# Symb0x76/ChineseChessZero

Measured on AMD Instinct MI355X. Metric: self-play MCTS simulations/sec, higher is better.
Workload: dtype u8 rules / f32 Q (reference CPU path) / f64 PUCT (net: fp16)

## Files before the change

chinesechesszero_amd/_lib.py:

```python
from __future__ import annotations

import ctypes as C
import os

import torch

_HERE = os.path.dirname(os.path.abspath(__file__))
LIB_PATH = os.path.join(_HERE, "libcczero.so")

NSQ = 90
SQ_STRIDE = 96
NMOVES = 2086
MAX_LEGAL = 128
MASK_WORDS = 66
PLANES = 10710
REC_BYTES, REC_HDR, REC_IDS, REC_PI = 880, 96, 112, 368
HEAD_POL_STRIDE, HEAD_VAL_STRIDE = 1536, 640

ABI_VERSION = 8
CONV_RELU, CONV_DESCENDING, CONV_FORCE_SMALL, CONV_FORCE_TILE, CONV_G16, CONV_G16_EDGE_TILES = 1, 2, 16, 32, 64, 128
CONV_G16_ONE_LAUNCH = 512
RULE_PERPETUAL_CHECK = 1
RULE_PAWN_MOVE_RESETS_CLOCK = 2
FLAG_REFERENCE_QUIRKS = 1
# ... 73 lines not shown
    "ccz_gather_priors_routed": (C.c_int, [_P, _P, _P, _P, C.c_int32, _P, _P]),
    "ccz_finish_move": (C.c_int, [_P, _P, _P, _P, _P, C.c_int32]),
    "ccz_root_children": (C.c_int, [_P, _P, _P, _P, _P, _P, _P, _P]),
    "ccz_principal_variations": (C.c_int, [_P, _P, C.c_int32, C.c_int32, _P, _P, _P, _P, _P, _P]),
    "ccz_root_pi": (C.c_int, [_P, _P, _P, _P]),
    "ccz_move_distribution": (C.c_int, [_P, _P, _P, _P, _P, _P]),
    "ccz_game_status": (C.c_int, [_P, _P, _P, _P, _P, _P]),
    "ccz_root_positions": (C.c_int, [_P, _P, _P]),
    "ccz_leaf_info": (C.c_int, [_P, _P, _P, _P, _P, _P]),
    "ccz_leaf_priors": (C.c_int, [_P, _P, _P, _P]),
    "ccz_leaf_keys": (C.c_int, [_P, _P, _P, _P]),
    "ccz_harvest_rows": (C.c_int, [_P, _P, C.POINTER(C.c_int64)]),
    "ccz_harvest": (C.c_int, [_P, _P, _P, _P, _P, C.c_int64, C.POINTER(C.c_int64)]),
    "ccz_harvest_records": (C.c_int, [_P, _P, _P, C.c_int64, C.POINTER(C.c_int64)]),
    "ccz_expand_records": (C.c_int, [_P, _P, C.c_int64, C.c_uint32, _P, _P, _P, _P, C.c_int64, C.c_int64, _P]),
    "ccz_ring_retire": (C.c_int, [_P, _P, C.c_int64, _P, C.c_int64, C.c_int32, _P]),
    "ccz_sample_records": (C.c_int, [_P, _P, C.c_int64, _P, _P, C.c_int64, C.c_uint32, _P, _P, _P, _P, _P]),
    "ccz_get_stats": (C.c_int, [_P, _P, C.POINTER(Stats)]),
    "ccz_legal_moves": (C.c_int, [_P, C.c_int32, _P, _P, _P, _P, _P, _P]),
    "ccz_apply_moves": (C.c_int, [_P, C.c_int32, _P, _P, _P, _P]),
    "ccz_bias_act_f16": (C.c_int, [_P, _P, _P, _P, C.c_int64, C.c_int32]),
    "ccz_conv3x3_c256_f16": (C.c_int, [_P, _P, _P, _P, _P, _P, C.c_int64, C.c_int32]),
    "ccz_conv3x3_stem_f16": (C.c_int, [_P, _P, _P, _P, _P, C.c_int64, C.c_int32]),
    "ccz_pack_live_planes_f16": (C.c_int, [_P, _P, _P, C.c_int32]),
    "ccz_pack_live_planes_rows_f16": (C.c_int, [_P, _P, _P, C.c_int32, _P, _P]),
    "ccz_pack_live_planes_g16_f16": (C.c_int, [_P, _P, _P, C.c_int32, _P, _P]),
    "ccz_pack_conv_weights_g16_f16": (C.c_int, [_P, _P, _P, C.c_int32]),
    "ccz_conv3x3_c256_f16_live": (C.c_int, [_P, _P, _P, _P, _P, _P, C.c_int64, C.c_int32, _P, C.c_int32, C.c_int32]),
    "ccz_conv3x3_stem_f16_live": (C.c_int, [_P, _P, _P, _P, _P, C.c_int64, C.c_int32, _P, C.c_int32, C.c_int32]),
    "ccz_conv3x3_c256_heads_f16": (C.c_int, [_P, _P, _P, _P, _P, _P, _P, _P, _P, C.c_int64, C.c_int32, _P, C.c_int32, C.c_int32]),
    "ccz_heads_conv1x1_f16": (C.c_int, [_P, _P, _P, _P, _P, _P, C.c_int32, C.c_int32, _P]),
    "ccz_fc_f16": (C.c_int, [_P, _P, C.c_int32, _P, _P, _P, C.c_int32, C.c_int32, C.c_int32, C.c_int32, C.c_int32, _P]),
    "ccz_value_out_f32": (C.c_int, [_P, _P, _P, C.c_float, _P, C.c_int32, _P]),
}

_lib = None


def source_hash() -> str | None:
    import glob
    import hashlib
    csrc = os.path.join(_HERE, "csrc")
    files = sorted(glob.glob(os.path.join(csrc, "*.h")) + glob.glob(os.path.join(csrc, "*.hip")), key=os.path.basename)
    files.append(os.path.join(os.path.dirname(_HERE), "include", "cczero.h"))
    if len(files) < 2 or not all(os.path.exists(f) for f in files):
        return None
    h = hashlib.sha256()
    for f in files:
        with open(f, "rb") as fh:
            h.update(fh.read())
    return h.hexdigest()[:16]


def stale_build() -> str | None:
    if LIB_PATH != os.path.join(_HERE, "libcczero.so"):
        return None
    want = source_hash()
    if want is None:
        return None
    stamp = LIB_PATH + ".srchash"
    if not os.path.exists(stamp):
        return f"{LIB_PATH} carries no source stamp ({stamp} is missing): it was not built by the current Makefile"
    with open(stamp) as f:
        got = f.read().strip()
    if got != want:
        return f"{LIB_PATH} was built from other sources (stamp {got}, the tree hashes to {want}): a kernel was edited after the last build"
# ... 28 lines not shown
```

chinesechesszero_amd/csrc/cczero.hip:

```cpp
#include "../../include/cczero.h"

#include <hip/hip_runtime.h>

#include <cmath>
#include <cstdarg>
#include <cstdio>
#include <cstring>
#include <new>
#include <vector>

#include "cczero_kernels.h"
#include "cczero_netops.h"
#include "cczero_conv.h"
#include "cczero_conv_small.h"
#include "cczero_conv_g16.h"
#include "cczero_conv_g16e.h"
#include "cczero_heads.h"

using namespace ccz;

namespace {

thread_local char g_err[512] = "";

// ... 1052 lines not shown
}

int ccz_conv3x3_c256_heads_f16(void *stream, const void *x_dev, const void *w_dev, const void *bias_f32_dev, const void *residual_dev,
                               const void *head_w32_dev, const void *head_b32_dev, void *pol_dev, void *val_dev, int64_t n_pixels, int32_t flags,
                               const int32_t *live_rows_dev, int32_t part, int32_t n_parts)
{
    const char *who = "ccz_conv3x3_c256_heads_f16";
    if (!x_dev || !w_dev || !bias_f32_dev || !residual_dev || !head_w32_dev || !head_b32_dev || !pol_dev || !val_dev || n_pixels < 0 || n_pixels % 1440 ||
        n_pixels > (int64_t)INT32_MAX / kCvC)
        return fail(-1, "%s: bad arguments (n_pixels must be a multiple of 16 boards * 90, at most 93200 boards per call)", who);
    if (!(flags & CCZ_CONV_G16)) return fail(-1, "%s: rows must be in the group-of-16 layout (CCZ_CONV_G16)", who);
    if ((((uintptr_t)x_dev) | ((uintptr_t)w_dev) | ((uintptr_t)bias_f32_dev) | ((uintptr_t)residual_dev) | ((uintptr_t)head_w32_dev) | ((uintptr_t)head_b32_dev)) & 15)
        return fail(-1, "%s: pointers must be 16-byte aligned", who);
    if ((((uintptr_t)pol_dev) | ((uintptr_t)val_dev)) & 1) return fail(-1, "%s: outputs must be 2-byte aligned", who);
    if (live_rows_dev && (n_parts < 1 || n_parts > 256 || part < 0 || part >= n_parts)) return fail(-1, "%s: bad part / n_parts", who);
    if (n_pixels == 0) return 0;
    const int groups = (int)(n_pixels / 1440);
    const int fl = flags & 3, row0 = live_rows_dev ? (part | (n_parts << 16)) : 0;
    G5Heads ha;
    ha.w32 = (const _Float16 *)head_w32_dev;
    ha.b32 = (const float *)head_b32_dev;
    ha.pol = (_Float16 *)pol_dev;
    ha.val = (_Float16 *)val_dev;
    ha.nb = (int)(n_pixels / 90);
    hipStream_t s = (hipStream_t)stream;
#define CCZ_G16H(KERNEL_, GRID_, FLAGS_)                                                                                                \
    hipLaunchKernelGGL(KERNEL_, dim3((unsigned)(GRID_)), dim3(512), 0, s, (const _Float16 *)x_dev, (const _Float16 *)w_dev, (const float *)bias_f32_dev, \
                       (const _Float16 *)residual_dev, (_Float16 *)nullptr, (int)n_pixels, (int)(FLAGS_), 256, (const int *)live_rows_dev, row0, ha)
    if (!(flags & CCZ_CONV_G16_EDGE_TILES) || groups < 2) {
        CCZ_G16H(k_conv3x3_g16_heads, groups * 5, fl);
        HIP_TRY(hipGetLastError());
        return 0;
    }
    CCZ_G16H(k_conv3x3_g16_heads, groups * 4, fl | 4);
    HIP_TRY(hipGetLastError());
    CCZ_G16H(k_conv3x3_g16_edge_heads, 2 * ((groups + 1) / 2), fl);
    HIP_TRY(hipGetLastError());
#undef CCZ_G16H
    return 0;
}

int ccz_conv3x3_stem_f16(void *stream, const void *x64_dev, const void *w_dev, const void *bias_f32_dev, void *y_dev, int64_t n_pixels, int32_t relu)
{
    return conv3x3_launch("ccz_conv3x3_stem_f16", stream, x64_dev, w_dev, bias_f32_dev, nullptr, y_dev, n_pixels, relu, 64);
}

int ccz_conv3x3_c256_f16_live(void *stream, const void *x_dev, const void *w_dev, const void *bias_f32_dev, const void *residual_dev, void *y_dev,
                              int64_t n_pixels, int32_t relu, const int32_t *live_rows_dev, int32_t part, int32_t n_parts)
{
    if (!live_rows_dev || n_parts < 1 || n_parts > 256 || part < 0 || part >= n_parts) return fail(-1, "ccz_conv3x3_c256_f16_live: null live-row count or bad part / n_parts");
    return conv3x3_launch("ccz_conv3x3_c256_f16_live", stream, x_dev, w_dev, bias_f32_dev, residual_dev, y_dev, n_pixels, relu, 256, live_rows_dev, part | (n_parts << 16));
}

int ccz_conv3x3_stem_f16_live(void *stream, const void *x64_dev, const void *w_dev, const void *bias_f32_dev, void *y_dev, int64_t n_pixels, int32_t relu,
                              const int32_t *live_rows_dev, int32_t part, int32_t n_parts)
{
    if (!live_rows_dev || n_parts < 1 || n_parts > 256 || part < 0 || part >= n_parts) return fail(-1, "ccz_conv3x3_stem_f16_live: null live-row count or bad part / n_parts");
    return conv3x3_launch("ccz_conv3x3_stem_f16_live", stream, x64_dev, w_dev, bias_f32_dev, nullptr, y_dev, n_pixels, relu, 64, live_rows_dev, part | (n_parts << 16));
}

int ccz_pack_live_planes_rows_f16(void *stream, const void *leaf_dev, void *x64_dev, int32_t n_boards, const int32_t *rows_dev, const int32_t *n_rows_dev)
{
    if (!leaf_dev || !x64_dev || n_boards < 0 || !rows_dev || !n_rows_dev) return fail(-1, "ccz_pack_live_planes_rows_f16: bad arguments");
    if ((uintptr_t)x64_dev & 15) return fail(-1, "ccz_pack_live_planes_rows_f16: output must be 16-byte aligned");
    if (n_boards == 0) return 0;
    hipLaunchKernelGGL(k_pack_live_planes, dim3((unsigned)n_boards), dim3(kPackThreads), 0, (hipStream_t)stream, (const _Float16 *)leaf_dev, (half8_t *)x64_dev, (int)n_boards,
// ... 84 lines not shown
        const dim3 wgrid((unsigned)(8 * ((wtiles + 7) / 8)));
        if (relu & 1)
            hipLaunchKernelGGL(k_fc_wide_f16<true>, wgrid, dim3(512), 0, (hipStream_t)stream, (const _Float16 *)a_dev, (int)lda, (const _Float16 *)w_dev,
                               (const float *)bias_f32_dev, (_Float16 *)c_dev, (int)ldc, (int)m, (int)n, (int)k, (const int *)live_rows_dev, (int)(relu >> 8));
        else
            hipLaunchKernelGGL(k_fc_wide_f16<false>, wgrid, dim3(512), 0, (hipStream_t)stream, (const _Float16 *)a_dev, (int)lda, (const _Float16 *)w_dev,
                               (const float *)bias_f32_dev, (_Float16 *)c_dev, (int)ldc, (int)m, (int)n, (int)k, (const int *)live_rows_dev, (int)(relu >> 8));
        HIP_TRY(hipGetLastError());
        return 0;
    }
    if (m <= 16 && !(relu & 6)) {
        const dim3 sgrid((unsigned)((n + 15) / 16));
        if (relu & 1)
            hipLaunchKernelGGL(k_fc_skinny_f16<true>, sgrid, dim3(64), 0, (hipStream_t)stream, (const _Float16 *)a_dev, (int)lda, (const _Float16 *)w_dev,
                               (const float *)bias_f32_dev, (_Float16 *)c_dev, (int)ldc, (int)m, (int)n, (int)k, (const int *)live_rows_dev);
        else
            hipLaunchKernelGGL(k_fc_skinny_f16<false>, sgrid, dim3(64), 0, (hipStream_t)stream, (const _Float16 *)a_dev, (int)lda, (const _Float16 *)w_dev,
                               (const float *)bias_f32_dev, (_Float16 *)c_dev, (int)ldc, (int)m, (int)n, (int)k, (const int *)live_rows_dev);
        HIP_TRY(hipGetLastError());
        return 0;
    }
    const int tiles = ((n + kFcBN - 1) / kFcBN) * ((m + kFcBM - 1) / kFcBM);
    const dim3 grid((unsigned)(8 * ((tiles + 7) / 8)));
    if (relu & 1)
        hipLaunchKernelGGL(k_fc_f16<true>, grid, dim3(256), 0, (hipStream_t)stream, (const _Float16 *)a_dev, (int)lda, (const _Float16 *)w_dev,
                           (const float *)bias_f32_dev, (_Float16 *)c_dev, (int)ldc, (int)m, (int)n, (int)k, (const int *)live_rows_dev, (int)(relu >> 8));
    else
        hipLaunchKernelGGL(k_fc_f16<false>, grid, dim3(256), 0, (hipStream_t)stream, (const _Float16 *)a_dev, (int)lda, (const _Float16 *)w_dev,
                           (const float *)bias_f32_dev, (_Float16 *)c_dev, (int)ldc, (int)m, (int)n, (int)k, (const int *)live_rows_dev, (int)(relu >> 8));
    HIP_TRY(hipGetLastError());
    return 0;
}

int ccz_value_out_f32(void *stream, const void *h_dev, const void *w2_dev, float b2, float *v_dev, int32_t m, const int32_t *live_rows_dev)
{
    if (!h_dev || !w2_dev || !v_dev || m < 0) return fail(-1, "ccz_value_out_f32: bad arguments");
    if ((((uintptr_t)h_dev) | ((uintptr_t)w2_dev)) & 7) return fail(-1, "ccz_value_out_f32: h and w2 must be 8-byte aligned");
    if (m == 0) return 0;
    hipLaunchKernelGGL(k_value_out, dim3((unsigned)((m + 3) / 4)), dim3(256), 0, (hipStream_t)stream, (const _Float16 *)h_dev, (const _Float16 *)w2_dev, b2, v_dev,
                       (int)m, (const int *)live_rows_dev);
    HIP_TRY(hipGetLastError());
    return 0;
}

}
```

chinesechesszero_amd/csrc/cczero_conv_g16e.h:

```cpp
#pragma once
#include "cczero_conv_g16.h"

namespace ccz {

__host__ __device__ constexpr int g5e_nslab(int h) { return h == 0 ? 2 : h == 1 ? 2 : h == 2 ? 1 : 0; }
__host__ __device__ constexpr int g5e_dma(int h) { return 2 + g5e_nslab(h); }
__host__ __device__ constexpr int g5e_vmcnt(int h) { return g5e_dma(h) + g5e_dma((h + 5) % 6); }
static_assert(g5e_vmcnt(0) == 6 && g5e_vmcnt(1) == 8 && g5e_vmcnt(2) == 7 && g5e_vmcnt(3) == 5 && g5e_vmcnt(4) == 4 && g5e_vmcnt(5) == 4, "g5e_vmcnt table");
static_assert(g5e_dma(0) == 4 && g5e_dma(1) == 4 && g5e_dma(2) == 3 && g5e_dma(3) == 2 && g5e_dma(4) == 2 && g5e_dma(5) == 2,
              "17 DMA loads per chunk and thread: 5 slab pieces + 6 x 2 weight pieces");

template <int J>
__device__ __forceinline__ void g5e_step(const G5Ctx &c, cv_f32x4 (&acc)[4][9], int chunk, int &ring_rd, int &ring_wr,
                                          cv_half8 (&a0)[4], cv_half8 (&a1)[4], cv_half8 (&b)[9], int toff)
{
    constexpr int H = J % 6, BUF = J / 6;
    constexpr int Hn = (H + 1) % 6, BUFn = (H == 5) ? 1 - BUF : BUF;
    cv_half8 (&acur)[4] = (J & 1) ? a1 : a0;
    cv_half8 (&anxt)[4] = (J & 1) ? a0 : a1;
    unsigned char *const lds = c.lds;
#define G5E_CELL(N)                                                                                                       \
    {                                                                                                                     \
        if constexpr (H % 3 == 2)                                                                                         \
            b[N] = *(const cv_half8 *)(lds + c.vb[BUFn] + ((Hn / 3) * 9 + N) * 1024);                                     \
// ... 206 lines not shown
__global__ __launch_bounds__(512) void k_conv3x3_g16_edge(const _Float16 *__restrict__ X, const _Float16 *__restrict__ W,
                                                            const float *__restrict__ bias, const _Float16 *R, _Float16 *Y, int M,
                                                            int relu, int cin, const int *live_rows, int row0)
{
    __shared__ __attribute__((aligned(16))) unsigned char lds[kG5Lds];
    g5e_tile<RES, false>(lds, blockIdx.x, X, W, bias, R, Y, M, relu, cin, live_rows, row0, G5Heads{});
}

__global__ __launch_bounds__(512) void k_conv3x3_g16_edge_heads(const _Float16 *__restrict__ X, const _Float16 *__restrict__ W,
                                                                  const float *__restrict__ bias, const _Float16 *R, _Float16 *Y,
                                                                  int M, int relu, int cin, const int *live_rows, int row0, G5Heads ha)
{
    __shared__ __attribute__((aligned(16))) unsigned char lds[kG5Lds];
    if (live_rows) ha.nb = *live_rows;
    g5e_tile<true, true>(lds, blockIdx.x, X, W, bias, R, Y, M, relu, cin, live_rows, row0, ha);
}

template <bool RES>
__global__ __launch_bounds__(512) void k_conv3x3_g16_one(const _Float16 *__restrict__ X, const _Float16 *__restrict__ W,
                                                           const float *__restrict__ bias, const _Float16 *R, _Float16 *Y, int M,
                                                           int relu, int cin, const int *live_rows, int row0)
{
    __shared__ __attribute__((aligned(16))) unsigned char lds[kG5Lds];
    int groups = M / 1440;
    if (live_rows) {
        int first;
        groups = g5_live_groups(live_rows, row0, groups, first);
    }
    const int mid = groups * 4, blk = blockIdx.x;
    if (blk < mid) g5_tile<RES, false>(lds, blk, mid, X, W, bias, R, Y, M, relu | 4, cin, live_rows, row0, G5Heads{});
    else g5e_tile<RES, false>(lds, blk - mid, X, W, bias, R, Y, M, relu, cin, live_rows, row0, G5Heads{});
}

}
```

chinesechesszero_amd/csrc/cczero_heads.h:

```cpp
#pragma once
#include <hip/hip_runtime.h>
#include <stdint.h>

#include "cczero_conv.h"
#include "cczero_device.h"

namespace ccz {

constexpr int kHdPol = 17, kHdVal = 7;
constexpr int kHdPolStride = 1536;
constexpr int kHdValStride = 640;

template <bool G16>
__global__ __launch_bounds__(256) void k_head_conv1x1(const _Float16 *__restrict__ X, const _Float16 *__restrict__ Wh,
                                                        const float *__restrict__ bh, _Float16 *__restrict__ pol,
                                                        _Float16 *__restrict__ val, int n_boards, const int *__restrict__ live)
{
    const int lane = threadIdx.x & 63, r = lane & 15, q4 = lane >> 4;
    const int wave = blockIdx.x * 4 + (threadIdx.x >> 6), n_waves = gridDim.x * 4;
    int nb = n_boards;
    if (live) { const int l = *live; nb = l < nb ? l : nb; }
    const long n_rows = G16 ? (long)((nb + 15) >> 4) * 1440 : (long)nb * 90;
    const int n_cells = (int)((n_rows + 15) >> 4);
    if (wave >= n_cells) return;
// ... 331 lines not shown
        }
        mfmas(fa1, fb1, s_ + 3, 0, s_ + 3 < ns ? 7 : 0);
    }
    FW_STAMP(2)
    if (FC_DBG(8)) { if (acc[0][0][0] == 12345.678f) C[0] = (_Float16)1; return; }
    __builtin_amdgcn_sched_barrier(0);
    __builtin_amdgcn_s_barrier();
    __builtin_amdgcn_sched_barrier(0);
    unsigned char *tb = lds + wv * (64 * kFwERow);
#pragma unroll
    for (int j = 0; j < 4; ++j)
#pragma unroll
        for (int i = 0; i < NF; ++i) {
            float v0 = acc[i][j][0], v1 = acc[i][j][1], v2 = acc[i][j][2], v3 = acc[i][j][3];
            if (RELU) { v0 = fmaxf(v0, 0.0f); v1 = fmaxf(v1, 0.0f); v2 = fmaxf(v2, 0.0f); v3 = fmaxf(v3, 0.0f); }
            cv_half4 o;
            o[0] = (_Float16)v0; o[1] = (_Float16)v1; o[2] = (_Float16)v2; o[3] = (_Float16)v3;
            *(cv_half4 *)(tb + (j * 16 + r) * kFwERow + (i * 16 + 4 * q4) * 2) = o;
        }
    wave_sync();
    constexpr int NW = NF * 8;
#pragma unroll 4
    for (int it = 0; it < NW; ++it) {
        const int L = it * 64 + lane, row = L / NW, dw = L - row * NW;
        const int m = m0 + wm * 64 + row, n = n0 + I0 * 16 + 2 * dw;
        const uint32_t v = *(const uint32_t *)(tb + row * kFwERow + dw * 4);
        if (m < Ml && n + 1 < N) *(uint32_t *)(C + (long)m * ldc + n) = v;
    }
    FW_STAMP(3)
#undef FW_STAMP
}

template <bool RELU>
__global__ __launch_bounds__(512) void k_fc_wide_f16(const _Float16 *__restrict__ A, int lda, const _Float16 *__restrict__ W,
                                                       const float *__restrict__ bias, _Float16 *__restrict__ C, int ldc, int M, int N,
                                                       int K, const int *__restrict__ live, [[maybe_unused]] int dbg)
{
    __shared__ __attribute__((aligned(16))) unsigned char lds[kFwStages * kFwStage];
    const int tid = threadIdx.x, lane = tid & 63;
    const int wv = __builtin_amdgcn_readfirstlane(tid >> 6), wm = wv & 3, wn = wv >> 2;
    int Ml = M;
    if (live) { const int l = *live; Ml = l < Ml ? l : Ml; }
    const int mt = (Ml + kFwBM - 1) / kFwBM, nt = (N + kFwBN - 1) / kFwBN, tiles = mt * nt;
    int n0, m0;
    {
        const int b = blockIdx.x, x = b & 7, per = tiles >> 3, rem = tiles & 7;
        if ((b >> 3) >= per + (x < rem ? 1 : 0)) return;
        const int t = x * per + (x < rem ? x : rem) + (b >> 3);
        const int full = (mt >> 1) * 2 * nt;
        const int blk = t < full ? t / (2 * nt) : (mt >> 1);
        const int r_ = t < full ? t % (2 * nt) : t - full;
        const int cnt = t < full ? 2 : 1;
        n0 = (r_ / cnt) * kFwBN;
        m0 = (2 * blk + r_ % cnt) * kFwBM;
    }
    const int wrows = ((N + 127) >> 7) << 7;
    const int c = (lane & 7) ^ ((4 * (wv & 1) + (lane >> 4)) & 7), lr = lane >> 3;
    const _Float16 *src[7];
#pragma unroll
    for (int t = 0; t < 4; ++t) {
        int m = m0 + (wv + 8 * t) * 8 + lr;
        m = m < Ml ? m : Ml - 1;
        src[t] = A + (long)m * lda + c * 8;
    }
#pragma unroll
    for (int t = 0; t < 3; ++t) {
        int n = n0 + (wv + 8 * t) * 8 + lr;
        n = n < wrows ? n : wrows - 1;
        src[4 + t] = W + (long)n * K + c * 8;
    }
    if (wn == 0) fw_wave<RELU, 5, 0>(lds, src, wv, wm, lane, bias, wrows - 4, C, ldc, Ml, N, K, m0, n0, dbg);
    else fw_wave<RELU, 4, 5>(lds, src, wv, wm, lane, bias, wrows - 4, C, ldc, Ml, N, K, m0, n0, dbg);
}

__global__ __launch_bounds__(256) void k_value_out(const _Float16 *__restrict__ h, const _Float16 *__restrict__ w2, float b2,
                                                    float *__restrict__ v, int M, const int *__restrict__ live)
{
    const int lane = threadIdx.x & 63, m = blockIdx.x * 4 + (threadIdx.x >> 6);
    if (m >= M) return;
    const cv_half4 x = *(const cv_half4 *)(h + (long)m * 256 + lane * 4), w = *(const cv_half4 *)(w2 + lane * 4);
    int Ml = M;
    if (live) { const int l = *live; Ml = l < Ml ? l : Ml; }
    if (m >= Ml) return;
    float s = (float)x[0] * (float)w[0];
    s += (float)x[1] * (float)w[1];
    s += (float)x[2] * (float)w[2];
    s += (float)x[3] * (float)w[3];
    s = wave_sum_f32(s) + b2;
    if (lane == 0) v[m] = tanhf((float)(_Float16)s);
}

}
```

chinesechesszero_amd/net.py:

```python
from __future__ import annotations

import os

import numpy as np
import torch
import torch.nn.functional as F
from torch import nn

PIECES = 7
PLAYS = 17


class ResBlock(nn.Module):

    def __init__(self, num_channels=256):
        super().__init__()
        self.conv1 = nn.Conv2d(num_channels, num_channels, kernel_size=(3, 3), stride=(1, 1), padding=1)
        self.conv1_bn = nn.BatchNorm2d(num_channels)
        self.conv1_act = nn.ReLU()
        self.conv2 = nn.Conv2d(num_channels, num_channels, kernel_size=(3, 3), stride=(1, 1), padding=1)
        self.conv2_bn = nn.BatchNorm2d(num_channels)
        self.conv2_act = nn.ReLU()

    def forward(self, x):
# ... 483 lines not shown
                            f"(k_conv3x3_g16 / k_conv3x3_small serve 256-channel towers): MIOpen convolutions + one-pass epilogue")
                for i in range(0, len(self.ws), 2):
                    y = self._epilogue(F.conv2d(x, self.ws[i], None, padding=1), self.bs[i])
                    x = self._epilogue(F.conv2d(y, self.ws[i + 1], None, padding=1), self.bs[i + 1], x)
        return self._heads(x, B, g16, plan, return_logits)

    def _fused_heads_ok(self, x) -> bool:
        return bool(self.opt.fused_heads and hasattr(self, "head_w32") and x.is_cuda and x.dtype == torch.float16 and x.shape[1] == 256
                    and x.is_contiguous(memory_format=torch.channels_last))

    def _head_buffers(self, Bx, dev):
        from . import _lib
        bufs = self.__dict__.setdefault("_head_bufs", {})
        key = (Bx, dev)
        if key not in bufs:
            bufs[key] = (torch.zeros((Bx, _lib.HEAD_POL_STRIDE), dtype=torch.float16, device=dev),
                         torch.zeros((Bx, _lib.HEAD_VAL_STRIDE), dtype=torch.float16, device=dev),
                         torch.empty((Bx, 256), dtype=torch.float16, device=dev))
        return bufs[key]

    def _heads_fused(self, x, B, g16, plan, conv_done=False):
        import ctypes as C
        from . import _lib
        L = _lib.lib()
        Bx, dev = x.shape[0], x.device
        pol, val, h1 = self._head_buffers(Bx, dev)
        logits = torch.empty((B, 2086), dtype=torch.float16, device=dev)
        v = torch.empty((B,), dtype=torch.float32, device=dev)
        s = C.c_void_p(torch.cuda.current_stream(dev).cuda_stream)
        live = C.c_void_p(plan[1].data_ptr()) if plan is not None else None
        P = lambda t: C.c_void_p(t.data_ptr())
        if not conv_done:
            _lib.check(L.ccz_heads_conv1x1_f16(s, P(x), P(self.head_w32), P(self.head_b32), P(pol), P(val), Bx, _lib.CONV_G16 if g16 else 0, live))
        _lib.check(L.ccz_fc_f16(s, P(pol), _lib.HEAD_POL_STRIDE, P(self.policy_fc_wp), P(self.policy_fc_b32), P(logits), 2086, B, 2086, 1536, 0, live))
        _lib.check(L.ccz_fc_f16(s, P(val), _lib.HEAD_VAL_STRIDE, P(self.value_fc1_wp), P(self.value_fc1_b32), P(h1), 256, B, 256, 640, 1, live))
        _lib.check(L.ccz_value_out_f32(s, P(h1), P(self.value_fc2_w), self._value_b2(), P(v), B, live))
        return logits, v

    def _value_b2(self) -> float:
        b2 = self.__dict__.get("_b2")
        if b2 is None:
            b2 = self.__dict__["_b2"] = float(self.value_fc2_b.detach().float().cpu().item())
        return b2

    def _heads(self, x, B, g16, plan, return_logits, conv_done=False):
        if self._fused_heads_ok(x):
            logits, v = self._heads_fused(x, B, g16, plan, conv_done)
            if return_logits:
                return logits, v
            return torch.exp(F.log_softmax(logits.float(), dim=1)).contiguous(), v
        Bx = x.shape[0]
        rows = x.permute(0, 2, 3, 1).reshape(Bx * 90, x.shape[1])
        h = F.relu_(torch.addmm(self.head_b, rows, self.head_wT))
        if g16:
            h = h.view(Bx // 16, 90, 16, PLAYS + PIECES).permute(0, 2, 1, 3).reshape(Bx, 90, PLAYS + PIECES)[:B]
        else:
            h = h.view(B, 90, PLAYS + PIECES)
        pol = h[:, :, :PLAYS].reshape(B, 90 * PLAYS)
        val = h[:, :, PLAYS:].reshape(B, 90 * PIECES)
        logits = F.linear(pol, self.policy_fc_w, self.policy_fc_b)
        v = F.relu_(F.linear(val, self.value_fc1_w, self.value_fc1_b))
        v = torch.tanh(F.linear(v, self.value_fc2_w, self.value_fc2_b).float()).view(B)
        if return_logits:
            return logits.contiguous(), v.contiguous()
        prob = torch.exp(F.log_softmax(logits.float(), dim=1))
        return prob.contiguous(), v.contiguous()
# ... 133 lines not shown
```

include/cczero.h:

```cpp
#ifndef CCZERO_H
#define CCZERO_H

#include <stdint.h>

#ifdef __cplusplus
extern "C" {
#endif

#define CCZ_ABI_VERSION 8
#define CCZ_NSQ 90
#define CCZ_SQ_STRIDE 96
#define CCZ_NMOVES 2086
#define CCZ_MAX_LEGAL 128
#define CCZ_MASK_WORDS 66
#define CCZ_PLANES 10710


#define CCZ_RULE_PAWN_MOVE_RESETS_CLOCK 2u
#define CCZ_RULE_PERPETUAL_CHECK 1u

#define CCZ_FLAG_REFERENCE_QUIRKS 1u
#define CCZ_FLAG_NO_MIRROR 2u
#define CCZ_FLAG_VALUE_F16 4u

// ... 164 lines not shown
#define CCZ_CONV_DESCENDING 2
#define CCZ_CONV_FORCE_SMALL 16
#define CCZ_CONV_FORCE_TILE 32
#define CCZ_CONV_G16 64
#define CCZ_CONV_G16_EDGE_TILES 128
#define CCZ_CONV_G16_ONE_LAUNCH 512
int ccz_conv3x3_c256_f16(void *stream, const void *x_dev, const void *w_dev, const void *bias_f32_dev,
                         const void *residual_dev, void *y_dev, int64_t n_pixels, int32_t relu);
int ccz_pack_conv_weights_g16_f16(void *stream, const void *w_dev, void *wp_dev, int32_t cin);

int ccz_conv3x3_stem_f16(void *stream, const void *x64_dev, const void *w_dev, const void *bias_f32_dev,
                         void *y_dev, int64_t n_pixels, int32_t relu);
int ccz_pack_live_planes_f16(void *stream, const void *leaf_dev, void *x64_dev, int32_t n_boards);
int ccz_pack_live_planes_g16_f16(void *stream, const void *leaf_dev, void *x64_dev, int32_t n_boards,
                                 const int32_t *rows_dev, const int32_t *n_rows_dev);

int ccz_pack_live_planes_rows_f16(void *stream, const void *leaf_dev, void *x64_dev, int32_t n_boards,
                                  const int32_t *rows_dev, const int32_t *n_rows_dev);
int ccz_conv3x3_c256_f16_live(void *stream, const void *x_dev, const void *w_dev, const void *bias_f32_dev,
                              const void *residual_dev, void *y_dev, int64_t n_pixels, int32_t relu,
                              const int32_t *live_rows_dev, int32_t part, int32_t n_parts);
int ccz_conv3x3_stem_f16_live(void *stream, const void *x64_dev, const void *w_dev, const void *bias_f32_dev,
                              void *y_dev, int64_t n_pixels, int32_t relu, const int32_t *live_rows_dev,
                              int32_t part, int32_t n_parts);

#define CCZ_HEAD_POL_STRIDE 1536
#define CCZ_HEAD_VAL_STRIDE 640
int ccz_heads_conv1x1_f16(void *stream, const void *x_dev, const void *w32_dev, const void *bias32_f32_dev, void *pol_dev,
                          void *val_dev, int32_t n_boards, int32_t flags, const int32_t *live_boards_dev);
int ccz_fc_f16(void *stream, const void *a_dev, int32_t lda, const void *w_dev, const void *bias_f32_dev, void *c_dev, int32_t ldc,
               int32_t m, int32_t n, int32_t k, int32_t relu, const int32_t *live_rows_dev);
int ccz_value_out_f32(void *stream, const void *h_dev, const void *w2_dev, float b2, float *v_dev, int32_t m,
                      const int32_t *live_rows_dev);

int ccz_conv3x3_c256_heads_f16(void *stream, const void *x_dev, const void *w_dev, const void *bias_f32_dev,
                               const void *residual_dev, const void *head_w32_dev, const void *head_bias32_f32_dev,
                               void *pol_dev, void *val_dev, int64_t n_pixels, int32_t flags,
                               const int32_t *live_rows_dev, int32_t part, int32_t n_parts);

#ifdef __cplusplus
}
#endif
#endif
```

profiles/summarize.py:

```python
#!/usr/bin/env python3
import csv
import glob
import json
import os
import sys
from collections import defaultdict


def find(d, pat):
    r = sorted(glob.glob(os.path.join(d, "**", pat), recursive=True))
    return r[0] if r else None


def main():
    out_dir, tag = sys.argv[1], sys.argv[2]
    root = os.path.dirname(os.path.abspath(__file__))
    summary = {}
    prev = os.path.join(root, f"{tag}_summary.json")
    if os.path.exists(prev):
        with open(prev) as f:
            summary = json.load(f)
    stats = find(os.path.join(out_dir, "trace"), "*kernel_stats.csv")
    if stats:
        rows = list(csv.DictReader(open(stats)))
        keep = rows[:48] + [r for r in rows[48:] if "ccz" in r.get("Name", "")]
        with open(os.path.join(root, f"{tag}_kernel_stats.csv"), "w", newline="") as f:
            w = csv.DictWriter(f, fieldnames=list(rows[0].keys()))
            w.writeheader()
            w.writerows(keep)
        for k in ("k_step", "k_softmax_gather", "k_select", "k_expand_backup", "k_finish_move", "k_harvest", "k_bias_act", "k_conv3x3"):
            hit = [r for r in rows if k in r.get("Name", "")]
            if hit:
                calls = sum(int(float(r.get("Calls", 0) or 0)) for r in hit)
                tot = sum(float(r.get("TotalDurationNs", 0) or 0) for r in hit)
                summary.setdefault(k, {})["avg_ns"] = tot / max(1, calls)
                summary[k]["calls"] = calls
                summary[k]["pct"] = sum(float(r.get("Percentage", 0) or 0) for r in hit)
                if len(hit) > 1:
                    summary[k]["variants"] = {r["Name"][:80]: {"calls": int(float(r["Calls"])), "avg_ns": float(r["AverageNs"])} for r in hit}
        plan_calls = sum(int(float(r.get("Calls", 0) or 0)) for r in rows if "k_cache_plan" in r.get("Name", ""))
        if plan_calls:
            tail = {}
            for k in ("k_cache_probe", "k_cache_plan", "k_pack_live_planes", "k_head_conv1x1", "k_fc_f16", "k_fc_wide_f16", "k_value_out", "k_softmax_gather"):
                tot = sum(float(r.get("TotalDurationNs", 0) or 0) for r in rows if k in r.get("Name", ""))
                calls = sum(int(float(r.get("Calls", 0) or 0)) for r in rows if k in r.get("Name", ""))
                if calls:
                    tail[k] = {"us_per_step": tot / plan_calls * 1e-3, "launches_per_step": calls / plan_calls, "avg_us": tot / calls * 1e-3}
            def fam(pred):
                hit = [r for r in rows if pred(r.get("Name", ""))]
                calls = sum(int(float(r.get("Calls", 0) or 0)) for r in hit)
                tot = sum(float(r.get("TotalDurationNs", 0) or 0) for r in hit)
                return calls, tot
            extra, detail = 0.0, {}
            for name, heads, plain in (("middle", lambda n: "k_conv3x3_g16_heads" in n, lambda n: "k_conv3x3_g16<true>" in n or "k_conv3x3_g16ILb1" in n),
                                       ("edge", lambda n: "k_conv3x3_g16_edge_heads" in n, lambda n: "k_conv3x3_g16_edge<true>" in n or "k_conv3x3_g16_edgeILb1" in n)):
                hc, ht = fam(heads)
                pc, pt = fam(plain)
                if hc and pc:
                    d = (ht / hc - pt / pc) * hc / plan_calls * 1e-3
                    extra += d
                    detail[name] = {"avg_us_with_heads": ht / hc * 1e-3, "avg_us_plain_residual_layer": pt / pc * 1e-3, "launches_per_step": hc / plan_calls, "extra_us_per_step": d}
            if detail:
                tail["heads_in_last_tower_layer"] = {"us_per_step": extra, "launches_per_step": sum(v["launches_per_step"] for v in detail.values()),
                                                     "avg_us": extra / max(1e-9, sum(v["launches_per_step"] for v in detail.values())), "detail": detail,
                                                     "what": "launch time of the last layer with the heads in its epilogue minus an ordinary residual layer's, x launches per step "
                                                             "(the chains run concurrently: an upper bound on what the step pays)"}
            other = [(r.get("Name", ""), float(r.get("TotalDurationNs", 0) or 0), int(float(r.get("Calls", 0) or 0))) for r in rows
                     if "ccz" not in r.get("Name", "")]
            summary["evaluator_tail"] = {"kernels": tail, "us_per_step_ours": sum(v["us_per_step"] for v in tail.values()),
                                         "library_kernels_total_us_per_step": sum(t for _, t, _ in other) / plan_calls * 1e-3,
                                         "library_kernels_top": [{"name": n[:90], "us_per_step": t / plan_calls * 1e-3, "calls": c} for n, t, c in sorted(other, key=lambda x: -x[1])[:8]],
                                         "steps": plan_calls,
                                         "what": "non-tower evaluator work per lockstep step (rocprofv3 --kernel-trace --stats of bench.py --steps 120): cache probe + plan, "
                                                 "pack of the live planes, head convolutions, FC layers, value head, softmax + gather + cache store. "
                                                 "library_kernels_*: kernels that are not this library's (torch elementwise / GEMM / copies), whole run "
                                                 "(set-up, preroll and the CPU-side bookkeeping included) divided by the number of steps"}
    def bench_line(name):
        p = os.path.join(out_dir, name)
        if not os.path.exists(p):
            return None
        try:
            return json.loads([l for l in open(p).read().splitlines() if l.startswith("{")][-1])
        except Exception:
            return None

    both_here = all(find(os.path.join(out_dir, k), "*counter_collection.csv") for k in ("pmc_fetch", "pmc_write"))
    if both_here:
        for key in ("k_bar", "d_bar", "warning"):
            summary.get("k_step", {}).get("window", {}).pop(key, None)
    for kind, counter in (("pmc_fetch", "FETCH_SIZE"), ("pmc_write", "WRITE_SIZE"), ("pmc_cfetch", "FETCH_SIZE"), ("pmc_cwrite", "WRITE_SIZE"),
                          ("pmc_hfetch", "FETCH_SIZE"), ("pmc_hwrite", "WRITE_SIZE")):
        cc = find(os.path.join(out_dir, kind), "*counter_collection.csv")
        if not cc:
            continue
        acc = defaultdict(lambda: [0.0, 0])
        kstep = []
        for r in csv.DictReader(open(cc)):
            if r.get("Counter_Name") != counter:
                continue
            name = r.get("Kernel_Name", "")
            for k in ("k_step", "k_softmax_gather", "k_select", "k_expand_backup", "k_finish_move", "k_conv3x3", "k_head_conv1x1", "k_fc_f16", "k_fc_wide_f16",
                      "k_pack_live_planes", "k_cache_plan", "k_cache_probe", "k_value_out"):
                if k in name:
                    acc[k][0] += float(r.get("Counter_Value", 0) or 0)
                    acc[k][1] += 1
                    if k == "k_step":
                        kstep.append((int(float(r.get("Dispatch_Id", 0) or 0)), float(r.get("Counter_Value", 0) or 0)))
        for k, (tot, n) in acc.items():
            if n:
                summary.setdefault(k, {})[counter + "_raw_per_launch"] = tot / n
                summary[k][counter + "_launches"] = n
        bl = bench_line(kind + "_bench.json")
        if bl and kstep and kind in ("pmc_fetch", "pmc_write"):
            n_win = int(bl["steps"]) - int(bl["move_boundary"]["in_window"])
            vals = [v for _, v in sorted(kstep, key=lambda t: t[0])][-n_win:]
            w = summary.setdefault("k_step", {}).setdefault("window", {})
            w[counter + "_raw_per_launch"] = sum(vals) / len(vals)
            w["launches"] = len(vals)
            rf = bl["roofline"]
            shape = {"k_bar": rf["k_bar"], "d_bar": rf["d_bar"], "algorithmic_bytes_per_launch": rf["algorithmic_bytes_per_launch"]}
            if "k_bar" in w and (abs(w["k_bar"] - shape["k_bar"]) > 1e-9 or abs(w["d_bar"] - shape["d_bar"]) > 1e-9):
                w["warning"] = f"the fetch and write passes saw different trees: {shape} vs k_bar {w['k_bar']} d_bar {w['d_bar']}"
            w.update(shape)
            w["bench_args"] = f"--steps {bl['steps']} --warmup {bl['warmup']} (window: {bl['config']['window']})"
    for sqdir in ("pmc_sq", "pmc_csq"):
      cc = find(os.path.join(out_dir, sqdir), "*counter_collection.csv")
      if cc:
          acc = defaultdict(lambda: defaultdict(lambda: [0.0, 0]))
          for r in csv.DictReader(open(cc)):
              name = r.get("Kernel_Name", "")
              for k in ("k_step", "k_softmax_gather", "k_finish_move", "k_harvest", "k_conv3x3"):
                  if k in name:
                      a = acc[k][r.get("Counter_Name")]
                      a[0] += float(r.get("Counter_Value", 0) or 0)
# ... 69 lines not shown
```

Measured before the change: 198,500.

## Fuse policy FC, value FC1 and value output into one tail kernel

Adds k_fc_tail_f16, which runs the policy FC tiles and a new value-head tile in one launch. The value tile computes FC1 with MFMA, applies ReLU into LDS and does the fc2 dot plus tanh in place, so h1 never goes to global memory. The three launches at the end of the evaluator become one, used when the batch is at least 2048. Also adds a one-launch variant of the heads conv layer that merges the middle and edge tiles, behind a flag. The cost is more complex kernels that share one LDS budget.

```diff
diff --git a/chinesechesszero_amd/_lib.py b/chinesechesszero_amd/_lib.py
--- a/chinesechesszero_amd/_lib.py
+++ b/chinesechesszero_amd/_lib.py
@@ -129,6 +129,8 @@
     "ccz_heads_conv1x1_f16": (C.c_int, [_P, _P, _P, _P, _P, _P, C.c_int32, C.c_int32, _P]),
     "ccz_fc_f16": (C.c_int, [_P, _P, C.c_int32, _P, _P, _P, C.c_int32, C.c_int32, C.c_int32, C.c_int32, C.c_int32, _P]),
     "ccz_value_out_f32": (C.c_int, [_P, _P, _P, C.c_float, _P, C.c_int32, _P]),
+    "ccz_fc_tail_f16": (C.c_int, [_P, _P, C.c_int32, _P, _P, _P, C.c_int32, C.c_int32, C.c_int32, _P, C.c_int32, _P, _P, C.c_int32, _P, C.c_float, _P,
+                                  C.c_int32, _P]),
 }
 
 _lib = None
diff --git a/chinesechesszero_amd/csrc/cczero.hip b/chinesechesszero_amd/csrc/cczero.hip
--- a/chinesechesszero_amd/csrc/cczero.hip
+++ b/chinesechesszero_amd/csrc/cczero.hip
@@ -1108,6 +1108,11 @@
         HIP_TRY(hipGetLastError());
         return 0;
     }
+    if (flags & CCZ_CONV_G16_ONE_LAUNCH) {
+        CCZ_G16H(k_conv3x3_g16_one_heads, groups * 4 + 2 * ((groups + 1) / 2), fl);
+        HIP_TRY(hipGetLastError());
+        return 0;
+    }
     CCZ_G16H(k_conv3x3_g16_heads, groups * 4, fl | 4);
     HIP_TRY(hipGetLastError());
     CCZ_G16H(k_conv3x3_g16_edge_heads, 2 * ((groups + 1) / 2), fl);
@@ -1258,6 +1263,37 @@
     return 0;
 }
 
+int ccz_fc_tail_f16(void *stream, const void *pol_dev, int32_t lda_pol, const void *wp_dev, const void *bp_f32_dev, void *logits_dev, int32_t ldc,
+                    int32_t n, int32_t k_pol, const void *val_dev, int32_t lda_val, const void *w1_dev, const void *b1_f32_dev, int32_t k_val,
+                    const void *w2_dev, float b2, float *v_dev, int32_t m, const int32_t *live_rows_dev)
+{
+    const char *who = "ccz_fc_tail_f16";
+    if (!pol_dev || !wp_dev || !bp_f32_dev || !logits_dev || !val_dev || !w1_dev || !b1_f32_dev || !w2_dev || !v_dev || m < 0 || n <= 0 || k_pol <= 0 || k_val <= 0)
+        return fail(-1, "%s: bad arguments", who);
+    if ((k_pol & 63) || (lda_pol & 7) || lda_pol < k_pol || (n & 1) || (ldc & 1) || ldc < n)
+        return fail(-1, "%s: k_pol must be a multiple of 64, lda_pol a multiple of 8 and >= k_pol, n and ldc even, ldc >= n", who);
+    if ((k_val & 63) || (lda_val & 7) || lda_val < k_val) return fail(-1, "%s: k_val must be a multiple of 64, lda_val a multiple of 8 and >= k_val", who);
+    if ((((uintptr_t)pol_dev) | ((uintptr_t)wp_dev) | ((uintptr_t)bp_f32_dev) | ((uintptr_t)val_dev) | ((uintptr_t)w1_dev) | ((uintptr_t)b1_f32_dev)) & 15)
+        return fail(-1, "%s: pol, val, the FC weights and biases must be 16-byte aligned", who);
+    if (((uintptr_t)logits_dev & 3) || ((uintptr_t)w2_dev & 7) || ((uintptr_t)v_dev & 3)) return fail(-1, "%s: logits and v must be 4-byte aligned, w2 8-byte aligned", who);
+    if (m == 0) return 0;
+    FcValue va;
+    va.a = (const _Float16 *)val_dev;
+    va.lda = (int)lda_val;
+    va.k = (int)k_val;
+    va.w1 = (const _Float16 *)w1_dev;
+    va.b1 = (const float *)b1_f32_dev;
+    va.w2 = (const _Float16 *)w2_dev;
+    va.b2 = b2;
+    va.v = v_dev;
+    const int wtiles = ((n + kFwBN - 1) / kFwBN) * ((m + kFwBM - 1) / kFwBM);
+    const dim3 grid((unsigned)((m + kFvBM - 1) / kFvBM + 8 * ((wtiles + 7) / 8)));
+    hipLaunchKernelGGL(k_fc_tail_f16, grid, dim3(512), 0, (hipStream_t)stream, (const _Float16 *)pol_dev, (int)lda_pol, (const _Float16 *)wp_dev,
+                       (const float *)bp_f32_dev, (_Float16 *)logits_dev, (int)ldc, (int)m, (int)n, (int)k_pol, (const int *)live_rows_dev, va);
+    HIP_TRY(hipGetLastError());
+    return 0;
+}
+
 int ccz_value_out_f32(void *stream, const void *h_dev, const void *w2_dev, float b2, float *v_dev, int32_t m, const int32_t *live_rows_dev)
 {
     if (!h_dev || !w2_dev || !v_dev || m < 0) return fail(-1, "ccz_value_out_f32: bad arguments");
diff --git a/chinesechesszero_amd/csrc/cczero_conv_g16e.h b/chinesechesszero_amd/csrc/cczero_conv_g16e.h
--- a/chinesechesszero_amd/csrc/cczero_conv_g16e.h
+++ b/chinesechesszero_amd/csrc/cczero_conv_g16e.h
@@ -262,4 +262,20 @@
     else g5e_tile<RES, false>(lds, blk - mid, X, W, bias, R, Y, M, relu, cin, live_rows, row0, G5Heads{});
 }
 
-}
+__global__ __launch_bounds__(512) void k_conv3x3_g16_one_heads(const _Float16 *__restrict__ X, const _Float16 *__restrict__ W,
+                                                                 const float *__restrict__ bias, const _Float16 *R, _Float16 *Y, int M,
+                                                                 int relu, int cin, const int *live_rows, int row0, G5Heads ha)
+{
+    __shared__ __attribute__((aligned(16))) unsigned char lds[kG5Lds];
+    int groups = M / 1440;
+    if (live_rows) {
+        int first;
+        groups = g5_live_groups(live_rows, row0, groups, first);
+        ha.nb = *live_rows;
+    }
+    const int mid = groups * 4, blk = blockIdx.x;
+    if (blk < mid) g5_tile<true, true>(lds, blk, mid, X, W, bias, R, Y, M, relu | 4, cin, live_rows, row0, ha);
+    else g5e_tile<true, true>(lds, blk - mid, X, W, bias, R, Y, M, relu, cin, live_rows, row0, ha);
+}
+
+}
diff --git a/chinesechesszero_amd/csrc/cczero_heads.h b/chinesechesszero_amd/csrc/cczero_heads.h
--- a/chinesechesszero_amd/csrc/cczero_heads.h
+++ b/chinesechesszero_amd/csrc/cczero_heads.h
@@ -387,19 +387,16 @@
 }
 
 template <bool RELU>
-__global__ __launch_bounds__(512) void k_fc_wide_f16(const _Float16 *__restrict__ A, int lda, const _Float16 *__restrict__ W,
-                                                       const float *__restrict__ bias, _Float16 *__restrict__ C, int ldc, int M, int N,
-                                                       int K, const int *__restrict__ live, [[maybe_unused]] int dbg)
-{
-    __shared__ __attribute__((aligned(16))) unsigned char lds[kFwStages * kFwStage];
+__device__ __forceinline__ void fw_tile(unsigned char *lds, int b, const _Float16 *__restrict__ A, int lda, const _Float16 *__restrict__ W,
+                                        const float *__restrict__ bias, _Float16 *__restrict__ C, int ldc, int Ml, int N, int K,
+                                        [[maybe_unused]] int dbg)
+{
     const int tid = threadIdx.x, lane = tid & 63;
     const int wv = __builtin_amdgcn_readfirstlane(tid >> 6), wm = wv & 3, wn = wv >> 2;
-    int Ml = M;
-    if (live) { const int l = *live; Ml = l < Ml ? l : Ml; }
     const int mt = (Ml + kFwBM - 1) / kFwBM, nt = (N + kFwBN - 1) / kFwBN, tiles = mt * nt;
     int n0, m0;
     {
-        const int b = blockIdx.x, x = b & 7, per = tiles >> 3, rem = tiles & 7;
+        const int x = b & 7, per = tiles >> 3, rem = tiles & 7;
         if ((b >> 3) >= per + (x < rem ? 1 : 0)) return;
         const int t = x * per + (x < rem ? x : rem) + (b >> 3);
         const int full = (mt >> 1) * 2 * nt;
@@ -428,6 +425,27 @@
     else fw_wave<RELU, 4, 5>(lds, src, wv, wm, lane, bias, wrows - 4, C, ldc, Ml, N, K, m0, n0, dbg);
 }
 
+template <bool RELU>
+__global__ __launch_bounds__(512) void k_fc_wide_f16(const _Float16 *__restrict__ A, int lda, const _Float16 *__restrict__ W,
+                                                       const float *__restrict__ bias, _Float16 *__restrict__ C, int ldc, int M, int N,
+                                                       int K, const int *__restrict__ live, [[maybe_unused]] int dbg)
+{
+    __shared__ __attribute__((aligned(16))) unsigned char lds[kFwStages * kFwStage];
+    int Ml = M;
+    if (live) { const int l = *live; Ml = l < Ml ? l : Ml; }
+    fw_tile<RELU>(lds, blockIdx.x, A, lda, W, bias, C, ldc, Ml, N, K, dbg);
+}
+
+__device__ __forceinline__ float value_out_row(const cv_half4 x, const cv_half4 w, float b2)
+{
+    float s = (float)x[0] * (float)w[0];
+    s += (float)x[1] * (float)w[1];
+    s += (float)x[2] * (float)w[2];
+    s += (float)x[3] * (float)w[3];
+    s = wave_sum_f32(s) + b2;
+    return (float)(_Float16)s;
+}
+
 __global__ __launch_bounds__(256) void k_value_out(const _Float16 *__restrict__ h, const _Float16 *__restrict__ w2, float b2,
                                                     float *__restrict__ v, int M, const int *__restrict__ live)
 {
@@ -437,12 +455,115 @@
     int Ml = M;
     if (live) { const int l = *live; Ml = l < Ml ? l : Ml; }
     if (m >= Ml) return;
-    float s = (float)x[0] * (float)w[0];
-    s += (float)x[1] * (float)w[1];
-    s += (float)x[2] * (float)w[2];
-    s += (float)x[3] * (float)w[3];
-    s = wave_sum_f32(s) + b2;
-    if (lane == 0) v[m] = tanhf((float)(_Float16)s);
-}
-
-}
+    const float t = value_out_row(x, w, b2);
+    if (lane == 0) v[m] = tanhf(t);
+}
+
+constexpr int kFvBM = 128, kFvHidden = 256;
+constexpr int kFvATile = kFvBM * 128, kFvStage = kFvATile + kFvHidden * 128;
+constexpr int kFvStages = 3;
+constexpr int kFvERow = kFvHidden * 2 + 16;
+static_assert(kFvStages * kFvStage <= kFwStages * kFwStage, "the value tile lives in the wide kernel's LDS");
+static_assert(kFvBM * kFvERow <= kFvStages * kFvStage, "the h1 image lives in the operand ring");
+
+struct FcValue {
+    const _Float16 *a;
+    int lda, k;
+    const _Float16 *w1;
+    const float *b1;
+    const _Float16 *w2;
+    float b2;
+    float *v;
+};
+
+__device__ __forceinline__ void fv_tile(unsigned char *lds, int b, const FcValue &va, int Ml)
+{
+    const int tid = threadIdx.x, lane = tid & 63, r = lane & 15, q4 = lane >> 4;
+    const int wv = __builtin_amdgcn_readfirstlane(tid >> 6), wn = wv & 3, wm = wv >> 2;
+    const int m0 = b * kFvBM;
+    const int c = (lane & 7) ^ ((4 * (wv & 1) + (lane >> 4)) & 7), lr = lane >> 3;
+    const _Float16 *src[6];
+#pragma unroll
+    for (int t = 0; t < 2; ++t) {
+        int m = m0 + (wv + 8 * t) * 8 + lr;
+        m = m < Ml ? m : Ml - 1;
+        src[t] = va.a + (long)m * va.lda + c * 8;
+    }
+#pragma unroll
+    for (int t = 0; t < 4; ++t) src[2 + t] = va.w1 + (long)((wv + 8 * t) * 8 + lr) * va.k + c * 8;
+    auto issue = [&](int st_) {
+        unsigned char *st = lds + (st_ % kFvStages) * kFvStage;
+#pragma unroll
+        for (int t = 0; t < 6; ++t) cv_glds16(src[t] + st_ * 64, st + (wv + 8 * t) * 1024);
+    };
+    cv_f32x4 acc[4][4];
+#pragma unroll
+    for (int i = 0; i < 4; ++i) {
+        const float4 bv = *(const float4 *)(va.b1 + wn * 64 + i * 16 + 4 * q4);
+#pragma unroll
+        for (int j = 0; j < 4; ++j) { acc[i][j][0] = bv.x; acc[i][j][1] = bv.y; acc[i][j][2] = bv.z; acc[i][j][3] = bv.w; }
+    }
+    const int ns = va.k / 64;
+    issue(0);
+    if (ns > 1) issue(1);
+    const int rsw = (r >> 1) & 7;
+    const int foff[2] = {r * 128 + ((q4 ^ rsw) << 4), r * 128 + (((4 + q4) ^ rsw) << 4)};
+    for (int s_ = 0; s_ < ns; ++s_) {
+        if (s_ + 1 < ns) cv_wait_vm<6>();
+        else cv_wait_vm<0>();
+        __builtin_amdgcn_sched_barrier(0);
+        __builtin_amdgcn_s_barrier();
+        __builtin_amdgcn_sched_barrier(0);
+        if (s_ + 2 < ns) issue(s_ + 2);
+        const unsigned char *base = lds + (s_ % kFvStages) * kFvStage;
+#pragma unroll
+        for (int ks = 0; ks < 2; ++ks) {
+            cv_half8 fa[4], fb[4];
+#pragma unroll
+            for (int j = 0; j < 4; ++j) fb[j] = *(const cv_half8 *)(base + (wm * 4 + j) * 2048 + foff[ks]);
+#pragma unroll
+            for (int i = 0; i < 4; ++i) fa[i] = *(const cv_half8 *)(base + kFvATile + (wn * 4 + i) * 2048 + foff[ks]);
+#pragma unroll
+            for (int i = 0; i < 4; ++i)
+#pragma unroll
+                for (int j = 0; j < 4; ++j) acc[i][j] = __builtin_amdgcn_mfma_f32_16x16x32_f16(fa[i], fb[j], acc[i][j], 0, 0, 0);
+        }
+    }
+    __builtin_amdgcn_sched_barrier(0);
+    __builtin_amdgcn_s_barrier();
+    __builtin_amdgcn_sched_barrier(0);
+#pragma unroll
+    for (int j = 0; j < 4; ++j)
+#pragma unroll
+        for (int i = 0; i < 4; ++i) {
+            cv_half4 o;
+            o[0] = (_Float16)fmaxf(acc[i][j][0], 0.0f); o[1] = (_Float16)fmaxf(acc[i][j][1], 0.0f);
+            o[2] = (_Float16)fmaxf(acc[i][j][2], 0.0f); o[3] = (_Float16)fmaxf(acc[i][j][3], 0.0f);
+            *(cv_half4 *)(lds + (wm * 64 + j * 16 + r) * kFvERow + (wn * 64 + i * 16 + 4 * q4) * 2) = o;
+        }
+    asm volatile("s_waitcnt lgkmcnt(0)" ::: "memory");
+    __builtin_amdgcn_sched_barrier(0);
+    __builtin_amdgcn_s_barrier();
+    __builtin_amdgcn_sched_barrier(0);
+    const cv_half4 w = *(const cv_half4 *)(va.w2 + lane * 4);
+    for (int it = 0; it < kFvBM / 8; ++it) {
+        const int row = wv * (kFvBM / 8) + it, m = m0 + row;
+        if (m >= Ml) break;
+        const float t = value_out_row(*(const cv_half4 *)(lds + row * kFvERow + lane * 8), w, va.b2);
+        if (lane == 0) va.v[m] = tanhf(t);
+    }
+}
+
+__global__ __launch_bounds__(512) void k_fc_tail_f16(const _Float16 *__restrict__ A, int lda, const _Float16 *__restrict__ W,
+                                                       const float *__restrict__ bias, _Float16 *__restrict__ C, int ldc, int M, int N,
+                                                       int K, const int *__restrict__ live, FcValue va)
+{
+    __shared__ __attribute__((aligned(16))) unsigned char lds[kFwStages * kFwStage];
+    int Ml = M;
+    if (live) { const int l = *live; Ml = l < Ml ? l : Ml; }
+    const int vt = (Ml + kFvBM - 1) / kFvBM, b = blockIdx.x;
+    if (b < vt) fv_tile(lds, b, va, Ml);
+    else fw_tile<false>(lds, b - vt, A, lda, W, bias, C, ldc, Ml, N, K, 0);
+}
+
+}
diff --git a/chinesechesszero_amd/net.py b/chinesechesszero_amd/net.py
--- a/chinesechesszero_amd/net.py
+++ b/chinesechesszero_amd/net.py
@@ -539,6 +539,11 @@
         P = lambda t: C.c_void_p(t.data_ptr())
         if not conv_done:
             _lib.check(L.ccz_heads_conv1x1_f16(s, P(x), P(self.head_w32), P(self.head_b32), P(pol), P(val), Bx, _lib.CONV_G16 if g16 else 0, live))
+        if B >= 2048:
+            _lib.check(L.ccz_fc_tail_f16(s, P(pol), _lib.HEAD_POL_STRIDE, P(self.policy_fc_wp), P(self.policy_fc_b32), P(logits), 2086, 2086, 1536,
+                                         P(val), _lib.HEAD_VAL_STRIDE, P(self.value_fc1_wp), P(self.value_fc1_b32), 640,
+                                         P(self.value_fc2_w), self._value_b2(), P(v), B, live))
+            return logits, v
         _lib.check(L.ccz_fc_f16(s, P(pol), _lib.HEAD_POL_STRIDE, P(self.policy_fc_wp), P(self.policy_fc_b32), P(logits), 2086, B, 2086, 1536, 0, live))
         _lib.check(L.ccz_fc_f16(s, P(val), _lib.HEAD_VAL_STRIDE, P(self.value_fc1_wp), P(self.value_fc1_b32), P(h1), 256, B, 256, 640, 1, live))
         _lib.check(L.ccz_value_out_f32(s, P(h1), P(self.value_fc2_w), self._value_b2(), P(v), B, live))
diff --git a/include/cczero.h b/include/cczero.h
--- a/include/cczero.h
+++ b/include/cczero.h
@@ -220,6 +220,10 @@
                int32_t m, int32_t n, int32_t k, int32_t relu, const int32_t *live_rows_dev);
 int ccz_value_out_f32(void *stream, const void *h_dev, const void *w2_dev, float b2, float *v_dev, int32_t m,
                       const int32_t *live_rows_dev);
+int ccz_fc_tail_f16(void *stream, const void *pol_dev, int32_t lda_pol, const void *wp_dev, const void *bp_f32_dev, void *logits_dev,
+                    int32_t ldc, int32_t n, int32_t k_pol, const void *val_dev, int32_t lda_val, const void *w1_dev,
+                    const void *b1_f32_dev, int32_t k_val, const void *w2_dev, float b2, float *v_dev, int32_t m,
+                    const int32_t *live_rows_dev);
 
 int ccz_conv3x3_c256_heads_f16(void *stream, const void *x_dev, const void *w_dev, const void *bias_f32_dev,
                                const void *residual_dev, const void *head_w32_dev, const void *head_bias32_f32_dev,
diff --git a/profiles/step_boundary.py b/profiles/step_boundary.py
--- /dev/null
+++ b/profiles/step_boundary.py
@@ -0,0 +1,142 @@
+import csv
+import json
+import re
+import sys
+
+import numpy as np
+
+import tower_tail
+
+MIN_US = 100.0
+
+
+TARG = {"Lb1E": "true", "Lb0E": "false", "DF16_": "_Float16", "f": "float"}
+
+
+def short(name):
+    m = re.match(r"_ZN3ccz(\d+)", name)
+    if m:
+        n = int(m.group(1))
+        base, rest = name[m.end():m.end() + n], name[m.end() + n:]
+        if rest.startswith("I"):
+            args, rest = [], rest[1:]
+            while rest and not rest.startswith("E"):
+                for k, v in TARG.items():
+                    if rest.startswith(k):
+                        args.append(v)
+                        rest = rest[len(k):]
+                        break
+                else:
+                    args.append("?")
+                    break
+            base += "<" + ",".join(args) + ">"
+        return base
+    name = re.sub(r"^void\s+", "", name.split("(")[0]).replace("ccz::", "")
+    name = re.sub(r"\s+", "", name)
+    return name if len(name) <= 72 else name[:69] + "..."
+
+
+def plain_layer(name):
+    return "k_conv3x3_g16" in name and "g16_stem" not in name and "heads" not in name
+
+
+def stat(v):
+    v = np.asarray(v, dtype=np.float64)
+    return {"median": round(float(np.median(v)), 2), "spread": round(float(v.max() - v.min()), 2)}
+
+
+def stat_mean(v):
+    v = np.asarray(v, dtype=np.float64)
+    return {**stat(v), "mean": round(float(v.mean()), 2), "std": round(float(v.std()), 2), "std_of_mean": round(float(v.std() / np.sqrt(len(v))), 2),
+            "p10": round(float(np.percentile(v, 10)), 2), "p90": round(float(np.percentile(v, 90)), 2)}
+
+
+def reduce(trace, bench):
+    line = json.loads([l for l in open(bench) if l.startswith("{")][-1])
+    ker, steps_t = [], []
+    with open(trace) as f:
+        for x in csv.DictReader(f):
+            s, e, name = int(x["Start_Timestamp"]), int(x["End_Timestamp"]), x["Kernel_Name"]
+            ker.append((s, e, name))
+            if "k_step" in name:
+                steps_t.append(s)
+    ker.sort()
+    steps_t.sort()
+    ms_step = line["ms_per_step"]
+    ok = [0.7 * ms_step < (b - a) / 1e6 < 1.4 * ms_step for a, b in zip(steps_t, steps_t[1:])]
+    end = max(i for i, v in enumerate(ok) if v) + 1
+    start = end
+    while start > 0 and ok[start - 1]:
+        start -= 1
+    t0, t1 = steps_t[start], steps_t[end]
+    steps = end - start
+    plain = [(s, min(e, t1)) for s, e, n in ker if plain_layer(n) and t0 <= s < t1]
+    free, cur = [], t0
+    for s, e in plain:
+        if s > cur:
+            free.append((cur, s))
+        cur = max(cur, e)
+    if t1 > cur:
+        free.append((cur, t1))
+    small_ns = sum(b - a for a, b in free if (b - a) / 1e3 <= MIN_US)
+    whole = [(a, b) for a, b in free if (b - a) / 1e3 > MIN_US and a > t0 and b < t1]
+    cut_ns = sum(b - a for a, b in free if (b - a) / 1e3 > MIN_US and not (a > t0 and b < t1))
+    others = [k for k in ker if not plain_layer(k[2])]
+    starts = np.array([k[0] for k in others])
+    items, sums, idle, ends = {}, [], [], []
+    for a, b in whole:
+        lo = np.searchsorted(starts, a - 2_000_000)
+        hi = np.searchsorted(starts, b)
+        seen, busy_to, nothing, end_of = {}, a, 0, {}
+        for s, e, name in others[lo:hi]:
+            if e <= a:
+                continue
+            n = short(name)
+            k = seen.get(n, 0)
+            seen[n] = k + 1
+            gap = max(0, s - busy_to) if s > a else 0
+            nothing += gap
+            busy_to = max(busy_to, e)
+            seg = "heads layer, all chains" if "heads" in n else "%s#%d" % (n, k)
+            end_of[seg] = max(end_of.get(seg, a), min(e, b))
+            it = items.setdefault("%s#%d" % (n, k), {"start": [], "end": [], "dur": [], "gap": []})
+            it["start"].append((s - a) / 1e3)
+            it["end"].append((e - a) / 1e3)
+            it["dur"].append((e - s) / 1e3)
+            it["gap"].append(gap / 1e3)
+        nothing += max(0, b - busy_to)
+        sums.append((b - a) / 1e3)
+        ends.append((end_of, a, b))
+        idle.append(nothing / 1e3)
+    n_b = len(whole)
+    rows = []
+    for key, it in items.items():
+        if len(it["start"]) * 2 < n_b:
+            continue
+        rows.append({"kernel": key, "in_boundaries": len(it["start"]), "start_us": stat(it["start"]), "end_us": stat(it["end"]),
+                     "duration_us": stat(it["dur"]), "gap_before_us": stat(it["gap"])})
+    rows.sort(key=lambda r: r["start_us"]["median"])
+    common = [k for k in {k for eo, _, _ in ends for k in eo} if sum(k in eo for eo, _, _ in ends) == len(ends)]
+    common.sort(key=lambda k: np.median([eo[k] - a for eo, a, _ in ends]))
+    segs = {k: [] for k in common + ["to the next step's first plain layer"]}
+    for eo, a, b in ends:
+        last = a
+        for k in common:
+            t = max(last, eo[k])
+            segs[k].append((t - last) / 1e3)
+            last = t
+        segs["to the next step's first plain layer"].append((b - last) / 1e3)
+    segments = [{"ends_with": k, **stat_mean(v)} for k, v in segs.items()]
+    tt = tower_tail.reduce(trace, bench, 1.0)["step_boundary_us_per_step"]
+    mine = (sum(b - a for a, b in whole) + cut_ns + small_ns) / 1e3 / steps
+    return {"sims_per_s": round(line["value"], 1), "ms_per_step": round(ms_step, 4), "code_hash": line.get("roofline", {}).get("code_hash"),
+            "steps_in_window": steps, "boundaries_itemised": n_b,
+            "sum_us": stat_mean(sums),
+            "nothing_in_flight_us": stat(idle),
+            "inside_tower_us_per_step": round(small_ns / 1e3 / steps, 2),
+            "check": {"tower_tail_step_boundary_us_per_step": tt, "this_reducer_us_per_step": round(mine, 1)},
+            "segments": segments, "kernels": rows}
+
+
+if __name__ == "__main__":
+    print(json.dumps(reduce(sys.argv[1], sys.argv[2]), indent=1))
diff --git a/profiles/summarize.py b/profiles/summarize.py
--- a/profiles/summarize.py
+++ b/profiles/summarize.py
@@ -41,7 +41,7 @@
         plan_calls = sum(int(float(r.get("Calls", 0) or 0)) for r in rows if "k_cache_plan" in r.get("Name", ""))
         if plan_calls:
             tail = {}
-            for k in ("k_cache_probe", "k_cache_plan", "k_pack_live_planes", "k_head_conv1x1", "k_fc_f16", "k_fc_wide_f16", "k_value_out", "k_softmax_gather"):
+            for k in ("k_cache_probe", "k_cache_plan", "k_pack_live_planes", "k_head_conv1x1", "k_fc_f16", "k_fc_wide_f16", "k_fc_tail_f16", "k_value_out", "k_softmax_gather"):
                 tot = sum(float(r.get("TotalDurationNs", 0) or 0) for r in rows if k in r.get("Name", ""))
                 calls = sum(int(float(r.get("Calls", 0) or 0)) for r in rows if k in r.get("Name", ""))
                 if calls:
@@ -53,7 +53,8 @@
                 return calls, tot
             extra, detail = 0.0, {}
             for name, heads, plain in (("middle", lambda n: "k_conv3x3_g16_heads" in n, lambda n: "k_conv3x3_g16<true>" in n or "k_conv3x3_g16ILb1" in n),
-                                       ("edge", lambda n: "k_conv3x3_g16_edge_heads" in n, lambda n: "k_conv3x3_g16_edge<true>" in n or "k_conv3x3_g16_edgeILb1" in n)):
+                                       ("edge", lambda n: "k_conv3x3_g16_edge_heads" in n, lambda n: "k_conv3x3_g16_edge<true>" in n or "k_conv3x3_g16_edgeILb1" in n),
+                                       ("one launch", lambda n: "k_conv3x3_g16_one_heads" in n, lambda n: "k_conv3x3_g16_one<true>" in n or "k_conv3x3_g16_oneILb1" in n)):
                 hc, ht = fam(heads)
                 pc, pt = fam(plain)
                 if hc and pc:
@@ -99,7 +100,7 @@
             if r.get("Counter_Name") != counter:
                 continue
             name = r.get("Kernel_Name", "")
-            for k in ("k_step", "k_softmax_gather", "k_select", "k_expand_backup", "k_finish_move", "k_conv3x3", "k_head_conv1x1", "k_fc_f16", "k_fc_wide_f16",
+            for k in ("k_step", "k_softmax_gather", "k_select", "k_expand_backup", "k_finish_move", "k_conv3x3", "k_head_conv1x1", "k_fc_f16", "k_fc_wide_f16", "k_fc_tail_f16",
                       "k_pack_live_planes", "k_cache_plan", "k_cache_probe", "k_value_out"):
                 if k in name:
                     acc[k][0] += float(r.get("Counter_Value", 0) or 0)
```

Result: no change. 199,600, median of 6 (+0.5%).
